# TheCacophonyProject/classifier-pipeline

Measured on AMD Instinct MI355X. Metric: CPTV frames/s end-to-end (track+classify) at 160x120, higher is better.
Workload: dtype u16/i32 track stage (f32 normalise, f64 gates); f32 crop/tile; f32 CNN (stride-1 3x3 convs of stages 2-4 (+ the stride-2 one): two fp16 planes per operand rounded to nearest (11 + 11 significand bits), power-of-two range scaling, 3 fp16 MFMAs per K step, device-side rerun in the exact split if an ac

## Files before the change

classifier-pipeline_amd/csrc/cpx_cnn_rw.hip:

```cpp
#include <hip/hip_runtime.h>

#include <algorithm>
#include <type_traits>

#include "cpx_conv_layout_core.h"
#include "cpx_kernels.h"

namespace cpx {

namespace {

typedef unsigned u32x4 __attribute__((ext_vector_type(4)));
typedef float f32x4 __attribute__((ext_vector_type(4)));
typedef _Float16 f16x2 __attribute__((ext_vector_type(2)));
typedef _Float16 f16x8 __attribute__((ext_vector_type(8)));

template <typename T>
__device__ __forceinline__ const T* at_off(const T* base, unsigned bytes) {
  return reinterpret_cast<const T*>(reinterpret_cast<const char*>(base) + bytes);
}
template <typename T>
__device__ __forceinline__ T* at_off(T* base, unsigned bytes) {
  return reinterpret_cast<T*>(reinterpret_cast<char*>(base) + bytes);
}
__device__ __forceinline__ unsigned pix_off(int y, int x, int W, int C) {
  return __umul24(__umul24((unsigned)y, (unsigned)W) + (unsigned)x, (unsigned)C);
}
__device__ __forceinline__ float relu_bits(float x) { return __int_as_float(max(__float_as_int(x), 0)); }
__device__ __forceinline__ void split_h(float a, float b, unsigned& hi, unsigned& lo) {
  f16x2 v = {(_Float16)a, (_Float16)b};
  hi = __builtin_bit_cast(unsigned, v);
  asm("v_fma_mixlo_f16 %0, %1, 1.0, -%2 op_sel:[0,0,0] op_sel_hi:[0,0,1]" : "=v"(lo) : "v"(a), "v"(hi));
  asm("v_fma_mixhi_f16 %0, %1, 1.0, -%2 op_sel:[0,0,1] op_sel_hi:[0,0,1]" : "+v"(lo) : "v"(b), "v"(hi));
}
__device__ __forceinline__ f32x4 mfma_h(u32x4 w, u32x4 x, f32x4 c) {
  return __builtin_amdgcn_mfma_f32_16x16x32_f16(__builtin_bit_cast(f16x8, w), __builtin_bit_cast(f16x8, x), c, 0, 0, 0);
}

struct RwTiles {
  unsigned long long m_tx, m_ty;
  int tiles_x, tiles_y, total;
};
template <int I, int N, typename F>
__device__ __forceinline__ void static_for(F&& f) {
  if constexpr (I < N) {
    f(std::integral_constant<int, I>{});
    static_for<I + 1, N>(f);
  }
}
__device__ __forceinline__ int div_magic(int n, unsigned long long m) { return (int)(((unsigned long long)n * m) >> 42); }

constexpr int RW_TW = 16;
constexpr int RW_CT = 256;
constexpr int RW_PPI = RW_CT / 8;
constexpr int RW_WC = 64;

template <int S, int NCH, int ROWS>
struct RwGeo {
  static constexpr int PW = 15 * S + 3, PH = (ROWS - 1) * S + 3, NPX = PH * PW;
  static constexpr int NP = (NPX * 8 + RW_CT - 1) / RW_CT;
  static constexpr int NPXP = (NP * RW_PPI + 3) / 4 * 4 + 2;
  static constexpr int BUF = 2 * 2 * NPXP * 2;
  static constexpr int STEPS = 3 * PH;
  static constexpr int CING = 32 * NCH;
  static constexpr size_t LDS = (size_t)2 * BUF * 16 + (size_t)(2 * CING + 3 * RW_WC) * sizeof(float);
};
constexpr int SC_NPXP = 258;
constexpr int SC_ITEMS = 16 * RW_TW * 8 / RW_CT;
constexpr size_t SC_LDS = (size_t)2 * 2 * SC_NPXP * 2 * 16;

template <int S, int NCH, int ROWS, bool BN, bool RES, bool SC = false>
__global__ __launch_bounds__(RW_CT) __attribute__((amdgpu_waves_per_eu(1, 1))) void conv_rw_kernel(ConvArgs a, const uint4* __restrict__ wimg, RwTiles td) {
  using G = RwGeo<S, NCH, ROWS>;
  constexpr int PW = G::PW, NPX = G::NPX, NP = G::NP, NPXP = G::NPXP, BUF = G::BUF, STEPS = G::STEPS, CING = G::CING, PH = G::PH;
  static_assert(!SC || (S == 1 && NCH == 2 && ROWS == 16 && !RES), "the fp16 shortcut is built into the stride-1 form's two-chunk stream");
  if (*a.ovf != 0) return;
  extern __shared__ __attribute__((aligned(16))) uint4 lds4[];
  uint4* s_buf = lds4;
  float* s_bn = reinterpret_cast<float*>(lds4 + 2 * BUF);
  float* s_par = s_bn + 2 * CING;
  uint4* s_sc = reinterpret_cast<uint4*>(s_par + 3 * RW_WC);
  const int tid = threadIdx.x, lane = tid & 63, wave = tid >> 6, i16 = lane & 15, q = lane >> 4;
  const int ct = wave;
  const int cout_g = a.Cout / a.groups, nhalf = cout_g / RW_WC;
  const int g = blockIdx.y / nhalf, half = blockIdx.y - g * nhalf;
  constexpr bool has_bn = BN;

  u32x4 Wr[NCH][9][2];
  {
    const u32x4* wg = reinterpret_cast<const u32x4*>(wimg) + (size_t)g * NCH * 3 * 24 * cout_g + (q * cout_g + half * RW_WC + ct * 16 + i16);
#pragma unroll
    for (int c = 0; c < NCH; ++c)
#pragma unroll
      for (int ky = 0; ky < 3; ++ky)
#pragma unroll
        for (int kx = 0; kx < 3; ++kx)
#pragma unroll
          for (int p = 0; p < 2; ++p) Wr[c][ky * 3 + kx][p] = wg[(size_t)((c * 3 + ky) * 24 + (p * 3 + kx) * 4) * cout_g];
  }
  u32x4 Wsc[2];
  if constexpr (SC) {
    const u32x4* ws = reinterpret_cast<const u32x4*>(a.sc_planes) + (size_t)g * 8 * cout_g + (q * cout_g + half * RW_WC + ct * 16 + i16);
    Wsc[0] = ws[0];
    Wsc[1] = ws[(size_t)4 * cout_g];
  }
  if (tid < CING) {
    const int ci = g * CING + tid;
    s_bn[tid] = has_bn ? a.in_scale[ci] * a.act_scale : a.act_scale;
    s_bn[CING + tid] = has_bn ? a.in_shift[ci] * a.act_scale : 0.0f;
  }
  if (tid < RW_WC) {
    const int ch = g * cout_g + half * RW_WC + tid;
    float os = a.w_unscale[ch] * a.act_unscale;
    if (a.out_scale) os *= a.out_scale[ch];
    float ob = a.out_shift ? a.out_shift[ch] : 0.0f;
    if (a.sc_in && a.sc_bias) ob += a.sc_bias[ch];
    s_par[tid] = os;
    s_par[RW_WC + tid] = ob;
    s_par[2 * RW_WC + tid] = a.w_scale[ch] * a.act_scale;
  }

  const int per_xcd = (td.total + 7) >> 3;
  auto tile_of = [&](int t) { return (t & 7) * per_xcd + (t >> 3); };
  auto decode = [&](int tile, int& n_, int& oy_, int& ox_) {
    int qd = div_magic(tile, td.m_tx);
    ox_ = (tile - qd * td.tiles_x) * RW_TW;
    tile = qd;
    qd = div_magic(tile, td.m_ty);
    oy_ = (tile - qd * td.tiles_y) * ROWS;
    n_ = qd;
  };
  int t = blockIdx.x;
  while (t < 8 * per_xcd && tile_of(t) >= td.total) t += gridDim.x;
  if (t >= 8 * per_xcd) return;
  auto advance = [&](int& n_, int& oy_, int& ox_) {
    t += gridDim.x;
    const bool more = t < 8 * per_xcd && tile_of(t) < td.total;
    if (more) decode(tile_of(t), n_, oy_, ox_);
    return more;
  };
  int n0, oy0, ox0, n1, oy1, ox1, n2, oy2, ox2;
  decode(tile_of(t), n0, oy0, ox0);

  u32x4 pre_p[NP];
  const int q8 = tid & 7;
  int ipos[NP];
#pragma unroll
  for (int i = 0; i < NP; ++i) {
    const int px = min((tid >> 3) + RW_PPI * i, NPX - 1);
    const int py = px / PW;
    ipos[i] = (py << 8) | (px - py * PW);
  }
  const unsigned st_base = (unsigned)((((q8 >> 2) * NPXP + (tid >> 3)) * 4 + (q8 & 3)) * 8);
  f32x4 psc[NCH], psh[NCH];
  const unsigned coff0 = (unsigned)(g * CING + 4 * q8);
  auto med3 = [](int x, int lo, int hi) __attribute__((always_inline)) {
    int r;
    asm("v_med3_i32 %0, %1, %2, %3" : "=v"(r) : "v"(x), "v"(lo), "s"(hi));
    return r;
  };
  const int Hm1 = a.H - 1, Wm1 = a.W - 1;
  auto issue_item = [&](const int i, const int c, const int n_, const int oy_, const int ox_) __attribute__((always_inline)) {
    const float* in_n = a.in + (size_t)n_ * a.H * a.W * a.Cin;
    const int iy = oy_ * S - a.pad_top + (ipos[i] >> 8), ix = ox_ * S - a.pad_left + (ipos[i] & 0xFF);
    const int cy = med3(iy, 0, Hm1), cx = med3(ix, 0, Wm1);
    pre_p[i] = *reinterpret_cast<const u32x4*>(at_off(in_n, (pix_off(cy, cx, a.W, a.Cin) + coff0 + (unsigned)(c * 32)) << 2));
  };
  unsigned hmax = 0u;
  auto pk_max_u16 = [](unsigned x, unsigned y) __attribute__((always_inline)) {
    unsigned r;
    asm("v_pk_max_u16 %0, %1, %2" : "=v"(r) : "v"(x), "v"(y));
    return r;
  };
  auto activate_item = [&](const int i, const int c, const int oy_, const int ox_) __attribute__((always_inline)) {
    float v[4];
#pragma unroll
    for (int j = 0; j < 4; ++j) v[j] = __fmaf_rn(__uint_as_float(pre_p[i][j]), psc[c][j], psh[c][j]);
    if (has_bn) {
#pragma unroll
      for (int j = 0; j < 4; ++j) v[j] = fmaxf(v[j], 0.0f);
    }
    const int iy = oy_ * S - a.pad_top + (ipos[i] >> 8), ix = ox_ * S - a.pad_left + (ipos[i] & 0xFF);
    const bool inside = (unsigned)iy < (unsigned)a.H && (unsigned)ix < (unsigned)a.W;
#pragma unroll
    for (int j = 0; j < 4; ++j) pre_p[i][j] = __float_as_uint(inside ? v[j] : 0.0f);
  };
  auto store_item = [&](const int i, const int bsel) __attribute__((always_inline)) {
    unsigned h0, h1, l0, l1;
    split_h(__uint_as_float(pre_p[i][0]), __uint_as_float(pre_p[i][1]), h0, l0);
    split_h(__uint_as_float(pre_p[i][2]), __uint_as_float(pre_p[i][3]), h1, l1);
    if (has_bn) hmax = pk_max_u16(pk_max_u16(hmax, h0), h1);
    else hmax = pk_max_u16(pk_max_u16(hmax, h0 & 0x7FFF7FFFu), h1 & 0x7FFF7FFFu);
    unsigned char* sp = reinterpret_cast<unsigned char*>(s_buf) + st_base;
    *reinterpret_cast<uint2*>(sp + (bsel * BUF * 16 + i * (RW_PPI * 32))) = make_uint2(h0, h1);
    *reinterpret_cast<uint2*>(sp + (bsel * BUF * 16 + 2 * NPXP * 32 + i * (RW_PPI * 32))) = make_uint2(l0, l1);
  };

  u32x4 pre_s[SC ? SC_ITEMS : 1];
  u32x4 xsh[2], xsl[2];
  const unsigned sc_st_base = (unsigned)((((q8 >> 2) * SC_NPXP + (tid >> 3)) * 4 + (q8 & 3)) * 8);
  const int sc_a_base = ((q >> 1) * SC_NPXP + i16) * 2 + (q & 1);
  auto issue_sc = [&](const int i, const int n_, const int oy_, const int ox_) __attribute__((always_inline)) {
    if constexpr (SC) {
      const float* sc_n = a.sc_in + (size_t)n_ * a.sc_H * a.sc_W * a.sc_cin;
      const int oy = min(oy_ + 2 * i + (tid >> 7), a.Ho - 1), ox = min(ox_ + ((tid >> 3) & 15), a.Wo - 1);
      pre_s[i] = *reinterpret_cast<const u32x4*>(
          at_off(sc_n, (pix_off(oy * a.sc_stride, ox * a.sc_stride, a.sc_W, a.sc_cin) + (unsigned)(g * 32 + 4 * q8)) << 2));
    }
  };
  auto store_sc = [&](const int i) __attribute__((always_inline)) {
    if constexpr (SC) {
      unsigned h0, h1, l0, l1;
      split_h(__uint_as_float(pre_s[i][0]) * a.sc_xscale, __uint_as_float(pre_s[i][1]) * a.sc_xscale, h0, l0);
      split_h(__uint_as_float(pre_s[i][2]) * a.sc_xscale, __uint_as_float(pre_s[i][3]) * a.sc_xscale, h1, l1);
      hmax = pk_max_u16(pk_max_u16(hmax, h0 & 0x7FFF7FFFu), h1 & 0x7FFF7FFFu);
      unsigned char* sp = reinterpret_cast<unsigned char*>(s_sc) + sc_st_base;
      *reinterpret_cast<uint2*>(sp + i * (RW_PPI * 32)) = make_uint2(h0, h1);
      *reinterpret_cast<uint2*>(sp + (2 * SC_NPXP * 32 + i * (RW_PPI * 32))) = make_uint2(l0, l1);
    }
  };

  f32x4 acc[ROWS];
  const int ch_l = g * cout_g + half * RW_WC + ct * 16 + 4 * q;
  auto init_acc = [&]() __attribute__((always_inline)) {
#pragma unroll
    for (int o = 0; o < ROWS; ++o) acc[o] = f32x4{0.0f, 0.0f, 0.0f, 0.0f};
  };
  f32x4 rres[RES ? ROWS : 1];
  auto issue_res = [&](const int o, const int n_, const int oy_, const int ox_) __attribute__((always_inline)) {
    if constexpr (RES) {
      const float* res_n = a.residual + (size_t)n_ * a.Ho * a.Wo * a.Cout;
      const int ox = min(ox_ + i16, a.Wo - 1), oy = min(oy_ + o, a.Ho - 1);
      rres[o] = *reinterpret_cast<const f32x4*>(at_off(res_n, (pix_off(oy, ox, a.Wo, a.Cout) + (unsigned)ch_l) << 2));
    }
  };

  const int a_base = ((q >> 1) * NPXP + S * i16) * 2 + (q & 1);
  constexpr int RW_AHEAD = 3, RW_RING = RW_AHEAD + 1;
  auto compute = [&](auto cc, auto bc, auto&& between) __attribute__((always_inline)) {
    constexpr int C = decltype(cc)::value, B = decltype(bc)::value;
    const uint4* sb = s_buf + B * BUF + a_base;
    u32x4 xh[RW_RING], xl[RW_RING];
    auto frag = [&](auto sc) __attribute__((always_inline)) {
      constexpr int s = decltype(sc)::value;
      constexpr int kx = s / PH, i = s - PH * kx, bf = s % RW_RING;
      xh[bf] = __builtin_bit_cast(u32x4, sb[(i * PW + kx) * 2]);
      xl[bf] = __builtin_bit_cast(u32x4, sb[4 * NPXP + (i * PW + kx) * 2]);
    };
    static_for<0, RW_AHEAD>(frag);
    static_for<0, STEPS>([&](auto sc) __attribute__((always_inline)) {
      constexpr int s = decltype(sc)::value;
      constexpr int kx = s / PH, i = s - PH * kx, bf = s % RW_RING;
      if constexpr (s + RW_AHEAD < STEPS) frag(std::integral_constant<int, s + RW_AHEAD>{});
      static_for<0, 3>([&](auto pc) __attribute__((always_inline)) {
        constexpr int pr = decltype(pc)::value;
        static_for<0, 3>([&](auto rc) __attribute__((always_inline)) {
          constexpr int r = decltype(rc)::value, d = i - r, o = d / S;
          if constexpr (d >= 0 && d % S == 0 && o < ROWS) {
            if constexpr (pr == 0) acc[o] = mfma_h(Wr[C][r * 3 + kx][1], xh[bf], acc[o]);
            if constexpr (pr == 1) acc[o] = mfma_h(Wr[C][r * 3 + kx][0], xl[bf], acc[o]);
            if constexpr (pr == 2) acc[o] = mfma_h(Wr[C][r * 3 + kx][0], xh[bf], acc[o]);
          }
        });
      });
      between(sc);
      __builtin_amdgcn_sched_barrier(0);
    });
  };
  auto unit = [&](auto cc, auto bc, auto ccc, auto cic, auto lastc, const int oyc, const int oxc, const int ni, const int oyi,
                  const int oxi) __attribute__((always_inline)) {
    constexpr int B = decltype(bc)::value, CC = decltype(ccc)::value, CI = decltype(cic)::value;
    constexpr bool LAST = decltype(lastc)::value;
    compute(cc, bc, [&](auto sc) __attribute__((always_inline)) {
      constexpr int s = decltype(sc)::value;
      constexpr int jlo = (s * 3 * NP + STEPS - 1) / STEPS, jhi = ((s + 1) * 3 * NP + STEPS - 1) / STEPS;
      static_for<jlo, (jhi < 3 * NP ? jhi : 3 * NP)>([&](auto jc) __attribute__((always_inline)) {
        constexpr int j = decltype(jc)::value, i = j / 3, k = j % 3;
        if constexpr (k == 0) activate_item(i, CC, oyc, oxc);
        if constexpr (k == 1) store_item(i, B ^ 1);
        if constexpr (k == 2) issue_item(i, CI, ni, oyi, oxi);
      });
      if constexpr (SC && !LAST) {
        constexpr int klo = (s * SC_ITEMS + STEPS - 1) / STEPS, khi = ((s + 1) * SC_ITEMS + STEPS - 1) / STEPS;
        static_for<klo, (khi < SC_ITEMS ? khi : SC_ITEMS)>([&](auto kc) __attribute__((always_inline)) { store_sc(decltype(kc)::value); });
      }
      if constexpr (SC && LAST) {
        if constexpr (s % 3 == 0 && s >= 3 && s / 3 - 1 < ROWS) {
          constexpr int o = s / 3 - 1;
          acc[o] = mfma_h(Wsc[1], xsh[o & 1], acc[o]);
          acc[o] = mfma_h(Wsc[0], xsl[o & 1], acc[o]);
          acc[o] = mfma_h(Wsc[0], xsh[o & 1], acc[o]);
        }
        if constexpr (s % 3 == 0 && s / 3 < ROWS) {
          constexpr int o = s / 3;
          xsh[o & 1] = __builtin_bit_cast(u32x4, s_sc[sc_a_base + o * 2 * RW_TW]);
          xsl[o & 1] = __builtin_bit_cast(u32x4, s_sc[sc_a_base + 4 * SC_NPXP + o * 2 * RW_TW]);
        }
        constexpr int klo = (s * SC_ITEMS + STEPS - 1) / STEPS, khi = ((s + 1) * SC_ITEMS + STEPS - 1) / STEPS;
        static_for<klo, (khi < SC_ITEMS ? khi : SC_ITEMS)>([&](auto kc) __attribute__((always_inline)) { issue_sc(decltype(kc)::value, ni, oyi, oxi); });
      }
      if constexpr (LAST && RES) {
        constexpr int olo = (s * ROWS + STEPS - 1) / STEPS, ohi = ((s + 1) * ROWS + STEPS - 1) / STEPS;
        static_for<olo, (ohi < ROWS ? ohi : ROWS)>([&](auto oc) __attribute__((always_inline)) { issue_res(decltype(oc)::value, n0, oy0, ox0); });
      }
    });
  };

  auto finish = [&](const int n_, const int oy_, const int ox_) __attribute__((always_inline)) {
    const int ox = min(ox_ + i16, a.Wo - 1);
    if (!SC && a.sc_in) {
      const int sc_cg = a.sc_cin / a.groups;
      const float* wsc = a.sc_w + ((size_t)g * sc_cg + q) * cout_g + half * RW_WC + ct * 16 + i16;
      const float ss = s_par[2 * RW_WC + ct * 16 + i16];
      const float* sc_n = a.sc_in + (size_t)n_ * a.sc_H * a.sc_W * a.sc_cin + g * sc_cg + q;
      for (int k4 = 0; k4 < sc_cg; k4 += 4) {
        const float ws = wsc[(size_t)k4 * cout_g] * ss;
#pragma unroll
        for (int o = 0; o < ROWS; ++o) {
          const int oy = min(oy_ + o, a.Ho - 1);
          const float xs = sc_n[((size_t)(oy * a.sc_stride) * a.sc_W + ox * a.sc_stride) * a.sc_cin + k4];
          acc[o] = __builtin_amdgcn_mfma_f32_16x16x4f32(ws, xs, acc[o], 0, 0, 0);
        }
      }
    }
    float* out_n = a.out + (size_t)n_ * a.Ho * a.Wo * a.Cout;
    const f32x4 os = *reinterpret_cast<const f32x4*>(s_par + ct * 16 + 4 * q);
    const f32x4 ob = *reinterpret_cast<const f32x4*>(s_par + RW_WC + ct * 16 + 4 * q);
    const bool xok = ox_ + i16 < a.Wo;
    const unsigned off0 = (pix_off(min(oy_, a.Ho - 1), ox, a.Wo, a.Cout) + (unsigned)ch_l) << 2;
    const unsigned row_bytes = (unsigned)(a.Wo * a.Cout) << 2;
    const bool whole = oy_ + ROWS <= a.Ho;
    auto row = [&](const int o, const bool ok, const unsigned off) __attribute__((always_inline)) {
      f32x4 v;
#pragma unroll
      for (int j = 0; j < 4; ++j) v[j] = __fmaf_rn(acc[o][j], os[j], ob[j]);
      if constexpr (RES) v += rres[o];
      if (a.relu) {
        asm volatile("");
        v.x = relu_bits(v.x); v.y = relu_bits(v.y); v.z = relu_bits(v.z); v.w = relu_bits(v.w);
      }
      if (ok) *reinterpret_cast<f32x4*>(at_off(out_n, off)) = v;
    };
    if (whole) {
#pragma unroll
      for (int o = 0; o < ROWS; ++o) row(o, xok, off0 + (unsigned)o * row_bytes);
    } else {
#pragma unroll
      for (int o = 0; o < ROWS; ++o) row(o, xok && oy_ + o < a.Ho, off0 + (unsigned)min(o, a.Ho - 1 - oy_) * row_bytes);
    }
  };

#pragma unroll
  for (int i = 0; i < NP; ++i) issue_item(i, 0, n0, oy0, ox0);
  __syncthreads();
#pragma unroll
  for (int c = 0; c < NCH; ++c) {
    psc[c] = *reinterpret_cast<const f32x4*>(s_bn + c * 32 + 4 * q8);
    psh[c] = *reinterpret_cast<const f32x4*>(s_bn + CING + c * 32 + 4 * q8);
  }
#pragma unroll
  for (int i = 0; i < NP; ++i) {
    activate_item(i, 0, oy0, ox0);
    store_item(i, 0);
  }
  using I0 = std::integral_constant<int, 0>;
  using I1 = std::integral_constant<int, 1>;
  using Yes = std::integral_constant<bool, true>;
  using No = std::integral_constant<bool, false>;
  if constexpr (NCH == 2) {
#pragma unroll
    for (int i = 0; i < NP; ++i) issue_item(i, 1, n0, oy0, ox0);
    if constexpr (SC) {
#pragma unroll
      for (int i = 0; i < SC_ITEMS; ++i) issue_sc(i, n0, oy0, ox0);
    }
    init_acc();
    for (;;) {
      n1 = n0; oy1 = oy0; ox1 = ox0;
      const bool more = advance(n1, oy1, ox1);
      __syncthreads();
      unit(I0{}, I0{}, I1{}, I0{}, No{}, oy0, ox0, n1, oy1, ox1);
      __syncthreads();
      unit(I1{}, I1{}, I0{}, I1{}, Yes{}, oy1, ox1, n1, oy1, ox1);
      finish(n0, oy0, ox0);
      if (!more) break;
      n0 = n1; oy0 = oy1; ox0 = ox1;
      init_acc();
    }
  } else {
    n1 = n0; oy1 = oy0; ox1 = ox0;
    bool more1 = advance(n1, oy1, ox1);
#pragma unroll
    for (int i = 0; i < NP; ++i) issue_item(i, 0, n1, oy1, ox1);
    init_acc();
    for (;;) {
      n2 = n1; oy2 = oy1; ox2 = ox1;
      bool more2 = more1 && advance(n2, oy2, ox2);
      __syncthreads();
      unit(I0{}, I0{}, I0{}, I0{}, Yes{}, oy1, ox1, n2, oy2, ox2);
      finish(n0, oy0, ox0);
      if (!more1) break;
      n0 = n1; oy0 = oy1; ox0 = ox1; n1 = n2; oy1 = oy2; ox1 = ox2; more1 = more2;
      init_acc();
      n2 = n1; oy2 = oy1; ox2 = ox1;
      more2 = more1 && advance(n2, oy2, ox2);
      __syncthreads();
      unit(I0{}, I1{}, I0{}, I0{}, Yes{}, oy1, ox1, n2, oy2, ox2);
      finish(n0, oy0, ox0);
      if (!more1) break;
      n0 = n1; oy0 = oy1; ox0 = ox1; n1 = n2; oy1 = oy2; ox1 = ox2; more1 = more2;
      init_acc();
    }
  }
  if ((hmax & 0x7FFFu) >= 0x7C00u || ((hmax >> 16) & 0x7FFFu) >= 0x7C00u) atomicOr(a.ovf, 1);
}

__global__ __launch_bounds__(256) void split_shortcut_kernel(const float* __restrict__ w, uint4* __restrict__ out, int groups, int cin_g,
                                                             int cout_g, const float* __restrict__ wscale, float factor) {
  const int nch = cin_g / 32;
  const int total = groups * nch * 4 * cout_g;
  const int idx = blockIdx.x * blockDim.x + threadIdx.x;
  if (idx >= total) return;
  const int col = idx % cout_g;
  int r = idx / cout_g;
  const int qq = r & 3;
  r >>= 2;
  const int chunk = r % nch, g = r / nch;
  const float f = wscale[g * cout_g + col] * factor;
  float v[8];
#pragma unroll
  for (int j = 0; j < 8; ++j) v[j] = w[((size_t)g * cin_g + chunk * 32 + 8 * qq + j) * cout_g + col] * f;
  uint4 hi, lo;
  split_h(v[0], v[1], hi.x, lo.x);
  split_h(v[2], v[3], hi.y, lo.y);
  split_h(v[4], v[5], hi.z, lo.z);
  split_h(v[6], v[7], hi.w, lo.w);
  const size_t base = (size_t)(g * nch + chunk) * 8 * cout_g + (size_t)qq * cout_g + col;
  out[base] = hi;
  out[base + (size_t)4 * cout_g] = lo;
}

}

bool conv_shortcut_planes_layer(const ConvArgs& second, int sc_cin_g) {
  if (conv_rw_kind(second) == 1) return sc_cin_g == 32;
  return second.ksize == 3 && second.stride == 1 && second.groups >= 1 && second.Cin == second.Cout &&
         second.Cout == 128 * second.groups && sc_cin_g == 64;
}
size_t conv_shortcut_image_bytes(int groups, int cin_g, int cout_g) { return (size_t)groups * (cin_g / 32) * 8 * cout_g * 16; }
void launch_split_shortcut(const float* sc_w, void* img, int groups, int cin_g, int cout_g, const float* w_scale, float factor,
                           hipStream_t s) {
  const int total = groups * (cin_g / 32) * 4 * cout_g;
  hipLaunchKernelGGL(split_shortcut_kernel, dim3((unsigned)((total + 255) / 256)), dim3(256), 0, s, sc_w, reinterpret_cast<uint4*>(img),
                     groups, cin_g, cout_g, w_scale, factor);
}

int conv_rw_kind(const ConvArgs& a) { return conv_rw_kind_of(conv_shape_of(a)); }
bool conv_rw_layer(const ConvArgs& a) { return conv_rw_kind(a) == 1; }

namespace {
template <int S, int NCH, int ROWS, bool BN, bool RES, bool SC = false>
int launch_rw_t(const ConvArgs& a, const uint4* wimg, hipStream_t s) {
  using G = RwGeo<S, NCH, ROWS>;
  constexpr size_t LDS = G::LDS + (SC ? SC_LDS : 0);
  static_assert(LDS <= 160 * 1024 - 1024, "two chunk buffers (and the shortcut's operand) must fit the CU's LDS");
  RwTiles td{};
  if (const int rc = fill_tiles(td, (a.Wo + RW_TW - 1) / RW_TW, (a.Ho + ROWS - 1) / ROWS, a.N, TILES_PERSISTENT)) return rc;
  static bool lds_ready[64];
  if (!cpx_dyn_lds_ready(reinterpret_cast<const void*>(conv_rw_kernel<S, NCH, ROWS, BN, RES, SC>), lds_ready, 160 * 1024 - 1024)) return -1;
  const int cus = cpx_device_cus();
  if (cus == 0) return -1;
  const int ny = a.groups * ((a.Cout / a.groups) / RW_WC);
  const int gx = persistent_grid_x(cus, ny, td.total);
  hipLaunchKernelGGL((conv_rw_kernel<S, NCH, ROWS, BN, RES, SC>), dim3((unsigned)gx, (unsigned)ny), dim3(RW_CT), LDS, s, a, wimg, td);
  return 0;
}
}

int launch_conv_rw(const ConvArgs& a, const void* wimg, hipStream_t s) {
  const int kind = conv_rw_kind(a);
  if (!kind || !a.half || a.planes != 2 || a.ovf == nullptr || a.in_planes || a.out_planes) return -2;
  if ((long long)a.H * a.W >= (1 << 24) || (long long)a.Ho * a.Wo >= (1 << 24)) return -3;
  if (a.sc_in && ((a.sc_cin / a.groups) & 3)) return -2;
  const uint4* wi = reinterpret_cast<const uint4*>(wimg);
  const bool bn = a.in_scale != nullptr, res = a.residual != nullptr;
  if (kind == 1) {
    if (a.pad_top != 1 || a.pad_left != 1 || a.H != a.Ho || a.W != a.Wo) return -2;
    if (a.sc_in && a.sc_planes) {
      if (bn || res || !conv_shortcut_planes_layer(a, a.sc_cin / a.groups) || a.sc_stride < 1 || !(a.sc_xscale > 0.0f) ||
          (a.sc_H - 1) / a.sc_stride + 1 != a.Ho || (a.sc_W - 1) / a.sc_stride + 1 != a.Wo)
        return -2;
      if ((long long)a.sc_H * a.sc_W >= (1 << 24) || (long long)a.sc_H * a.sc_W * a.sc_cin >= (1ll << 30)) return -3;
      return launch_rw_t<1, 2, 16, false, false, true>(a, wi, s);
    }
    if (bn && res) return launch_rw_t<1, 2, 16, true, true>(a, wi, s);
    if (bn) return launch_rw_t<1, 2, 16, true, false>(a, wi, s);
    if (res) return launch_rw_t<1, 2, 16, false, true>(a, wi, s);
    return launch_rw_t<1, 2, 16, false, false>(a, wi, s);
  }
  if (res || a.sc_in || a.pad_top < 0 || a.pad_top > 1 || a.pad_left < 0 || a.pad_left > 1) return -2;
  if (kind == 2) return bn ? launch_rw_t<2, 1, 8, true, false>(a, wi, s) : launch_rw_t<2, 1, 8, false, false>(a, wi, s);
  return bn ? launch_rw_t<3, 2, 4, true, false>(a, wi, s) : launch_rw_t<3, 2, 4, false, false>(a, wi, s);
}

}
```

classifier-pipeline_amd/csrc/cpx_conv_layout_core.h:

```cpp
#pragma once
#include <stddef.h>

#include <algorithm>

namespace cpx {

struct ConvShape { int groups, cin_g, cout_g, ksize, stride; };
template <class Args>
ConvShape conv_shape_of(const Args& a) {
  if (a.groups < 1 || a.Cin % a.groups || a.Cout % a.groups) return ConvShape{};
  return ConvShape{a.groups, a.Cin / a.groups, a.Cout / a.groups, a.ksize, a.stride};
}

enum class ConvClass { Unsupported, Plain, Flat, Wide, C8, Stride2Rw, Rw3 };

inline ConvClass conv_class(const ConvShape& s) {
  if (s.ksize != 3) return ConvClass::Unsupported;
  if (s.stride == 3 && s.cin_g == 64 && s.cout_g == 128) return ConvClass::Rw3;
  if (s.stride == 2 && s.cin_g == 32 && s.cout_g == 64) return ConvClass::Stride2Rw;
  if (s.stride == 1 && s.cin_g == 8 && s.cout_g == 32) return ConvClass::C8;
  const bool c32_64 = s.cout_g == 32 || s.cout_g == 64;
  if (s.stride == 1 && (s.cin_g == 32 || s.cin_g == 64) && c32_64) return ConvClass::Wide;
  if (s.cin_g < 16 || s.cin_g % 16) return ConvClass::Unsupported;
  if ((s.stride == 1 && s.cout_g == 128) || (s.stride == 2 && s.cout_g == 64)) return ConvClass::Flat;
  return s.stride == 1 && c32_64 ? ConvClass::Plain : ConvClass::Unsupported;
}
inline int conv_rw_kind_of(const ConvShape& s) {
  switch (conv_class(s)) {
    case ConvClass::Wide: return s.cin_g == 64 && s.cout_g == 64 ? 1 : 0;
    case ConvClass::Stride2Rw: return 2;
    case ConvClass::Rw3: return 3;
    default: return 0;
  }
}

struct WeightImages {
  static constexpr size_t absent = ~(size_t)0;
  static constexpr size_t C8_HALF_ENTRIES = 3 * 2 * 4 * 32;
  ConvClass cls = ConvClass::Unsupported;
  int chunk = 0;
  size_t planes3 = absent, planes2 = absent, half = absent, scales = absent, rw_half = absent, bytes = 0;

  static WeightImages of(const ConvShape& s) {
    WeightImages l;
    l.cls = conv_class(s);
    if (l.cls == ConvClass::Unsupported) return l;
    const auto put = [&l](size_t& image, size_t size) { image = l.bytes; l.bytes += size; };
    const size_t row = (size_t)s.cout_g * 16;
    const size_t scales = ((size_t)2 * s.groups * s.cout_g * sizeof(float) + 15) / 16 * 16;
    if (l.cls == ConvClass::C8) {
      put(l.planes3, (size_t)s.groups * 30 * row);
      put(l.half, (size_t)s.groups * C8_HALF_ENTRIES * 16);
      put(l.scales, scales);
      return l;
    }
    l.chunk = l.cls == ConvClass::Wide || l.cls == ConvClass::Rw3 ? 32 : 16;
    const auto image = [&](int planes) { return (size_t)s.groups * (s.cin_g / l.chunk) * (9 * l.chunk / 8 * planes) * row; };
    if (l.cls != ConvClass::Rw3) put(l.planes3, image(3));
    if (l.cls == ConvClass::Plain) return l;
    if (l.cls != ConvClass::Rw3) put(l.planes2, image(2));
    put(l.half, image(2));
    put(l.scales, scales);
    if (l.cls == ConvClass::Stride2Rw) put(l.rw_half, image(2));
    return l;
  }
};

constexpr int TILE_AXIS_LIMIT = 4096;
constexpr long long TILES_PER_LAUNCH = 1ll << 22;
constexpr long long TILES_PERSISTENT = (1ll << 22) - 8;
inline unsigned long long tile_magic(int d) { return (1ull << 42) / (unsigned long long)d + 1; }

template <class Tiles>
int fill_tiles(Tiles& td, int tiles_x, int tiles_y, long long n, long long limit) {
  if (tiles_x < 1 || tiles_y < 1 || tiles_x >= TILE_AXIS_LIMIT || tiles_y >= TILE_AXIS_LIMIT) return -3;
  const long long total = (long long)tiles_x * tiles_y * n;
  if (total >= limit) return -3;
  td.tiles_x = tiles_x, td.m_tx = tile_magic(tiles_x);
  td.tiles_y = tiles_y, td.m_ty = tile_magic(tiles_y);
  td.total = (int)total;
  return 0;
}
template <class Tiles>
int fill_tiles(Tiles& td, int tiles_x, int tiles_y, long long n, int nsplit, long long limit) {
  if (nsplit < 1 || nsplit >= TILE_AXIS_LIMIT) return -3;
  td.nsplit = nsplit, td.m_nsplit = tile_magic(nsplit);
  return fill_tiles(td, tiles_x, tiles_y, n * nsplit, limit);
}

inline int persistent_grid_x(int cus, int ny, long long tiles) {
  const int gx = std::max(8, cus / std::max(ny, 1) / 8 * 8);
  return (int)std::min<long long>(gx, (tiles + 7) / 8 * 8);
}

}
```

Before: 3.106 million.

## Give each wave two output-channel tiles in the stride-3 row-window conv

For the stride-3 layer (64->128 channels), each wave now computes two 16-channel output tiles, so one block covers all 128 channels and each staged input fragment feeds twice as many MFMAs. This halves the grid in y and removes the duplicate input staging and fp16 splitting across blocks. To keep register pressure manageable it shortens the fragment prefetch ring, issues fragment loads after the products, and computes item positions arithmetically. It also adds a CPX_RW_GRID environment override for the persistent grid size. The risk is higher VGPR use (doubled weight and accumulator registers) and fewer blocks in flight.

```diff
diff --git a/classifier-pipeline_amd/csrc/cpx_cnn_rw.hip b/classifier-pipeline_amd/csrc/cpx_cnn_rw.hip
--- a/classifier-pipeline_amd/csrc/cpx_cnn_rw.hip
+++ b/classifier-pipeline_amd/csrc/cpx_cnn_rw.hip
@@ -1,6 +1,7 @@
 #include <hip/hip_runtime.h>
 
 #include <algorithm>
+#include <cstdlib>
 #include <type_traits>
 
 #include "cpx_conv_layout_core.h"
@@ -63,7 +64,8 @@
   static constexpr int BUF = 2 * 2 * NPXP * 2;
   static constexpr int STEPS = 3 * PH;
   static constexpr int CING = 32 * NCH;
-  static constexpr size_t LDS = (size_t)2 * BUF * 16 + (size_t)(2 * CING + 3 * RW_WC) * sizeof(float);
+  static constexpr int CTW = S == 3 ? 2 : 1, WC = RW_WC * CTW;
+  static constexpr size_t LDS = (size_t)2 * BUF * 16 + (size_t)(2 * CING + 3 * WC) * sizeof(float);
 };
 constexpr int SC_NPXP = 258;
 constexpr int SC_ITEMS = 16 * RW_TW * 8 / RW_CT;
@@ -73,34 +75,38 @@
 __global__ __launch_bounds__(RW_CT) __attribute__((amdgpu_waves_per_eu(1, 1))) void conv_rw_kernel(ConvArgs a, const uint4* __restrict__ wimg, RwTiles td) {
   using G = RwGeo<S, NCH, ROWS>;
   constexpr int PW = G::PW, NPX = G::NPX, NP = G::NP, NPXP = G::NPXP, BUF = G::BUF, STEPS = G::STEPS, CING = G::CING, PH = G::PH;
+  constexpr int CTW = G::CTW, WC = G::WC;
+  static_assert(CTW == 1 || (!RES && !SC), "two channel tiles per wave: the stride-3 layer has neither residual nor shortcut");
   static_assert(!SC || (S == 1 && NCH == 2 && ROWS == 16 && !RES), "the fp16 shortcut is built into the stride-1 form's two-chunk stream");
   if (*a.ovf != 0) return;
   extern __shared__ __attribute__((aligned(16))) uint4 lds4[];
   uint4* s_buf = lds4;
   float* s_bn = reinterpret_cast<float*>(lds4 + 2 * BUF);
   float* s_par = s_bn + 2 * CING;
-  uint4* s_sc = reinterpret_cast<uint4*>(s_par + 3 * RW_WC);
+  uint4* s_sc = reinterpret_cast<uint4*>(s_par + 3 * WC);
   const int tid = threadIdx.x, lane = tid & 63, wave = tid >> 6, i16 = lane & 15, q = lane >> 4;
-  const int ct = wave;
-  const int cout_g = a.Cout / a.groups, nhalf = cout_g / RW_WC;
+  const int ct = wave * CTW;
+  const int cout_g = a.Cout / a.groups, nhalf = cout_g / WC;
   const int g = blockIdx.y / nhalf, half = blockIdx.y - g * nhalf;
   constexpr bool has_bn = BN;
 
-  u32x4 Wr[NCH][9][2];
+  u32x4 Wr[CTW][NCH][9][2];
   {
-    const u32x4* wg = reinterpret_cast<const u32x4*>(wimg) + (size_t)g * NCH * 3 * 24 * cout_g + (q * cout_g + half * RW_WC + ct * 16 + i16);
-#pragma unroll
-    for (int c = 0; c < NCH; ++c)
-#pragma unroll
-      for (int ky = 0; ky < 3; ++ky)
-#pragma unroll
-        for (int kx = 0; kx < 3; ++kx)
-#pragma unroll
-          for (int p = 0; p < 2; ++p) Wr[c][ky * 3 + kx][p] = wg[(size_t)((c * 3 + ky) * 24 + (p * 3 + kx) * 4) * cout_g];
+    const u32x4* wg = reinterpret_cast<const u32x4*>(wimg) + (size_t)g * NCH * 3 * 24 * cout_g + (q * cout_g + half * WC + ct * 16 + i16);
+#pragma unroll
+    for (int w = 0; w < CTW; ++w)
+#pragma unroll
+      for (int c = 0; c < NCH; ++c)
+#pragma unroll
+        for (int ky = 0; ky < 3; ++ky)
+#pragma unroll
+          for (int kx = 0; kx < 3; ++kx)
+#pragma unroll
+            for (int p = 0; p < 2; ++p) Wr[w][c][ky * 3 + kx][p] = wg[(size_t)((c * 3 + ky) * 24 + (p * 3 + kx) * 4) * cout_g + w * 16];
   }
   u32x4 Wsc[2];
   if constexpr (SC) {
-    const u32x4* ws = reinterpret_cast<const u32x4*>(a.sc_planes) + (size_t)g * 8 * cout_g + (q * cout_g + half * RW_WC + ct * 16 + i16);
+    const u32x4* ws = reinterpret_cast<const u32x4*>(a.sc_planes) + (size_t)g * 8 * cout_g + (q * cout_g + half * WC + ct * 16 + i16);
     Wsc[0] = ws[0];
     Wsc[1] = ws[(size_t)4 * cout_g];
   }
@@ -109,15 +115,15 @@
     s_bn[tid] = has_bn ? a.in_scale[ci] * a.act_scale : a.act_scale;
     s_bn[CING + tid] = has_bn ? a.in_shift[ci] * a.act_scale : 0.0f;
   }
-  if (tid < RW_WC) {
-    const int ch = g * cout_g + half * RW_WC + tid;
+  if (tid < WC) {
+    const int ch = g * cout_g + half * WC + tid;
     float os = a.w_unscale[ch] * a.act_unscale;
     if (a.out_scale) os *= a.out_scale[ch];
     float ob = a.out_shift ? a.out_shift[ch] : 0.0f;
     if (a.sc_in && a.sc_bias) ob += a.sc_bias[ch];
     s_par[tid] = os;
-    s_par[RW_WC + tid] = ob;
-    s_par[2 * RW_WC + tid] = a.w_scale[ch] * a.act_scale;
+    s_par[WC + tid] = ob;
+    s_par[2 * WC + tid] = a.w_scale[ch] * a.act_scale;
   }
 
   const int per_xcd = (td.total + 7) >> 3;
@@ -144,26 +150,36 @@
 
   u32x4 pre_p[NP];
   const int q8 = tid & 7;
-  int ipos[NP];
-#pragma unroll
-  for (int i = 0; i < NP; ++i) {
-    const int px = min((tid >> 3) + RW_PPI * i, NPX - 1);
-    const int py = px / PW;
-    ipos[i] = (py << 8) | (px - py * PW);
-  }
+  constexpr bool IPOS3 = S == 3;
+  static_assert(!IPOS3 || (PW == 48 && RW_PPI == 32 && NP * RW_PPI == NPX), "item i = pixel (tid >> 3) + 32 i of a 48-pixel row, none past the patch");
+  int ipos[IPOS3 ? 2 : NP];
+  if constexpr (IPOS3) {
+    const int px0 = tid >> 3;
+    ipos[0] = px0;
+    ipos[1] = px0 < 16 ? px0 + 32 : (1 << 8) | (px0 - 16);
+  } else {
+#pragma unroll
+    for (int i = 0; i < NP; ++i) {
+      const int px = min((tid >> 3) + RW_PPI * i, NPX - 1);
+      const int py = px / PW;
+      ipos[i] = (py << 8) | (px - py * PW);
+    }
+  }
+  auto item_pos = [&](const int i) __attribute__((always_inline)) { return IPOS3 ? ipos[i % 3 == 1] + ((2 * i / 3) << 8) + (i % 3 == 2 ? 16 : 0) : ipos[i]; };
   const unsigned st_base = (unsigned)((((q8 >> 2) * NPXP + (tid >> 3)) * 4 + (q8 & 3)) * 8);
   f32x4 psc[NCH], psh[NCH];
   const unsigned coff0 = (unsigned)(g * CING + 4 * q8);
-  auto med3 = [](int x, int lo, int hi) __attribute__((always_inline)) {
+  auto clamp0 = [](int x, int hi) __attribute__((always_inline)) {
     int r;
-    asm("v_med3_i32 %0, %1, %2, %3" : "=v"(r) : "v"(x), "v"(lo), "s"(hi));
+    asm("v_med3_i32 %0, %1, 0, %2" : "=v"(r) : "v"(x), "s"(hi));
     return r;
   };
   const int Hm1 = a.H - 1, Wm1 = a.W - 1;
   auto issue_item = [&](const int i, const int c, const int n_, const int oy_, const int ox_) __attribute__((always_inline)) {
     const float* in_n = a.in + (size_t)n_ * a.H * a.W * a.Cin;
-    const int iy = oy_ * S - a.pad_top + (ipos[i] >> 8), ix = ox_ * S - a.pad_left + (ipos[i] & 0xFF);
-    const int cy = med3(iy, 0, Hm1), cx = med3(ix, 0, Wm1);
+    const int ip = item_pos(i);
+    const int iy = oy_ * S - a.pad_top + (ip >> 8), ix = ox_ * S - a.pad_left + (ip & 0xFF);
+    const int cy = clamp0(iy, Hm1), cx = clamp0(ix, Wm1);
     pre_p[i] = *reinterpret_cast<const u32x4*>(at_off(in_n, (pix_off(cy, cx, a.W, a.Cin) + coff0 + (unsigned)(c * 32)) << 2));
   };
   unsigned hmax = 0u;
@@ -180,20 +196,21 @@
 #pragma unroll
       for (int j = 0; j < 4; ++j) v[j] = fmaxf(v[j], 0.0f);
     }
-    const int iy = oy_ * S - a.pad_top + (ipos[i] >> 8), ix = ox_ * S - a.pad_left + (ipos[i] & 0xFF);
+    const int ip = item_pos(i);
+    const int iy = oy_ * S - a.pad_top + (ip >> 8), ix = ox_ * S - a.pad_left + (ip & 0xFF);
     const bool inside = (unsigned)iy < (unsigned)a.H && (unsigned)ix < (unsigned)a.W;
 #pragma unroll
     for (int j = 0; j < 4; ++j) pre_p[i][j] = __float_as_uint(inside ? v[j] : 0.0f);
   };
-  auto store_item = [&](const int i, const int bsel) __attribute__((always_inline)) {
+  auto store_item = [&](const int i, const unsigned boff) __attribute__((always_inline)) {
     unsigned h0, h1, l0, l1;
     split_h(__uint_as_float(pre_p[i][0]), __uint_as_float(pre_p[i][1]), h0, l0);
     split_h(__uint_as_float(pre_p[i][2]), __uint_as_float(pre_p[i][3]), h1, l1);
     if (has_bn) hmax = pk_max_u16(pk_max_u16(hmax, h0), h1);
     else hmax = pk_max_u16(pk_max_u16(hmax, h0 & 0x7FFF7FFFu), h1 & 0x7FFF7FFFu);
     unsigned char* sp = reinterpret_cast<unsigned char*>(s_buf) + st_base;
-    *reinterpret_cast<uint2*>(sp + (bsel * BUF * 16 + i * (RW_PPI * 32))) = make_uint2(h0, h1);
-    *reinterpret_cast<uint2*>(sp + (bsel * BUF * 16 + 2 * NPXP * 32 + i * (RW_PPI * 32))) = make_uint2(l0, l1);
+    *reinterpret_cast<uint2*>(sp + (boff + i * (RW_PPI * 32))) = make_uint2(h0, h1);
+    *reinterpret_cast<uint2*>(sp + (boff + 2 * NPXP * 32 + i * (RW_PPI * 32))) = make_uint2(l0, l1);
   };
 
   u32x4 pre_s[SC ? SC_ITEMS : 1];
@@ -220,11 +237,13 @@
     }
   };
 
-  f32x4 acc[ROWS];
-  const int ch_l = g * cout_g + half * RW_WC + ct * 16 + 4 * q;
+  f32x4 acc[CTW][ROWS];
+  const int ch_l = g * cout_g + half * WC + ct * 16 + 4 * q;
   auto init_acc = [&]() __attribute__((always_inline)) {
 #pragma unroll
-    for (int o = 0; o < ROWS; ++o) acc[o] = f32x4{0.0f, 0.0f, 0.0f, 0.0f};
+    for (int w = 0; w < CTW; ++w)
+#pragma unroll
+      for (int o = 0; o < ROWS; ++o) acc[w][o] = f32x4{0.0f, 0.0f, 0.0f, 0.0f};
   };
   f32x4 rres[RES ? ROWS : 1];
   auto issue_res = [&](const int o, const int n_, const int oy_, const int ox_) __attribute__((always_inline)) {
@@ -236,9 +255,28 @@
   };
 
   const int a_base = ((q >> 1) * NPXP + S * i16) * 2 + (q & 1);
-  constexpr int RW_AHEAD = 3, RW_RING = RW_AHEAD + 1;
+  constexpr bool FRAG_AFTER = CTW == 2;
+  constexpr int RW_AHEAD = S == 3 ? 2 : 3, RW_RING = FRAG_AFTER ? RW_AHEAD : RW_AHEAD + 1;
+  auto products = [&](auto cc, auto sc, const u32x4& h, const u32x4& l) __attribute__((always_inline)) {
+    constexpr int C = decltype(cc)::value, s = decltype(sc)::value;
+    constexpr int kx = s / PH, i = s - PH * kx;
+    static_for<0, 3>([&](auto pc) __attribute__((always_inline)) {
+      constexpr int pr = decltype(pc)::value;
+      static_for<0, 3>([&](auto rc) __attribute__((always_inline)) {
+        constexpr int r = decltype(rc)::value, d = i - r, o = d / S;
+        if constexpr (d >= 0 && d % S == 0 && o < ROWS) {
+          static_for<0, CTW>([&](auto wc) __attribute__((always_inline)) {
+            constexpr int w = decltype(wc)::value;
+            if constexpr (pr == 0) acc[w][o] = mfma_h(Wr[w][C][r * 3 + kx][1], h, acc[w][o]);
+            if constexpr (pr == 1) acc[w][o] = mfma_h(Wr[w][C][r * 3 + kx][0], l, acc[w][o]);
+            if constexpr (pr == 2) acc[w][o] = mfma_h(Wr[w][C][r * 3 + kx][0], h, acc[w][o]);
+          });
+        }
+      });
+    });
+  };
   auto compute = [&](auto cc, auto bc, auto&& between) __attribute__((always_inline)) {
-    constexpr int C = decltype(cc)::value, B = decltype(bc)::value;
+    constexpr int B = decltype(bc)::value;
     const uint4* sb = s_buf + B * BUF + a_base;
     u32x4 xh[RW_RING], xl[RW_RING];
     auto frag = [&](auto sc) __attribute__((always_inline)) {
@@ -250,19 +288,10 @@
     static_for<0, RW_AHEAD>(frag);
     static_for<0, STEPS>([&](auto sc) __attribute__((always_inline)) {
       constexpr int s = decltype(sc)::value;
-      constexpr int kx = s / PH, i = s - PH * kx, bf = s % RW_RING;
-      if constexpr (s + RW_AHEAD < STEPS) frag(std::integral_constant<int, s + RW_AHEAD>{});
-      static_for<0, 3>([&](auto pc) __attribute__((always_inline)) {
-        constexpr int pr = decltype(pc)::value;
-        static_for<0, 3>([&](auto rc) __attribute__((always_inline)) {
-          constexpr int r = decltype(rc)::value, d = i - r, o = d / S;
-          if constexpr (d >= 0 && d % S == 0 && o < ROWS) {
-            if constexpr (pr == 0) acc[o] = mfma_h(Wr[C][r * 3 + kx][1], xh[bf], acc[o]);
-            if constexpr (pr == 1) acc[o] = mfma_h(Wr[C][r * 3 + kx][0], xl[bf], acc[o]);
-            if constexpr (pr == 2) acc[o] = mfma_h(Wr[C][r * 3 + kx][0], xh[bf], acc[o]);
-          }
-        });
-      });
+      constexpr int bf = s % RW_RING;
+      if constexpr (!FRAG_AFTER && s + RW_AHEAD < STEPS) frag(std::integral_constant<int, s + RW_AHEAD>{});
+      products(cc, sc, xh[bf], xl[bf]);
+      if constexpr (FRAG_AFTER && s + RW_AHEAD < STEPS) frag(std::integral_constant<int, s + RW_AHEAD>{});
       between(sc);
       __builtin_amdgcn_sched_barrier(0);
     });
@@ -271,13 +300,17 @@
                   const int oxi) __attribute__((always_inline)) {
     constexpr int B = decltype(bc)::value, CC = decltype(ccc)::value, CI = decltype(cic)::value;
     constexpr bool LAST = decltype(lastc)::value;
+    if constexpr (CTW == 2) {
+      psc[CC] = *reinterpret_cast<const f32x4*>(s_bn + CC * 32 + 4 * q8);
+      psh[CC] = *reinterpret_cast<const f32x4*>(s_bn + CING + CC * 32 + 4 * q8);
+    }
     compute(cc, bc, [&](auto sc) __attribute__((always_inline)) {
       constexpr int s = decltype(sc)::value;
       constexpr int jlo = (s * 3 * NP + STEPS - 1) / STEPS, jhi = ((s + 1) * 3 * NP + STEPS - 1) / STEPS;
       static_for<jlo, (jhi < 3 * NP ? jhi : 3 * NP)>([&](auto jc) __attribute__((always_inline)) {
         constexpr int j = decltype(jc)::value, i = j / 3, k = j % 3;
         if constexpr (k == 0) activate_item(i, CC, oyc, oxc);
-        if constexpr (k == 1) store_item(i, B ^ 1);
+        if constexpr (k == 1) store_item(i, (unsigned)((B ^ 1) * BUF * 16));
         if constexpr (k == 2) issue_item(i, CI, ni, oyi, oxi);
       });
       if constexpr (SC && !LAST) {
@@ -287,9 +320,9 @@
       if constexpr (SC && LAST) {
         if constexpr (s % 3 == 0 && s >= 3 && s / 3 - 1 < ROWS) {
           constexpr int o = s / 3 - 1;
-          acc[o] = mfma_h(Wsc[1], xsh[o & 1], acc[o]);
-          acc[o] = mfma_h(Wsc[0], xsl[o & 1], acc[o]);
-          acc[o] = mfma_h(Wsc[0], xsh[o & 1], acc[o]);
+          acc[0][o] = mfma_h(Wsc[1], xsh[o & 1], acc[0][o]);
+          acc[0][o] = mfma_h(Wsc[0], xsl[o & 1], acc[0][o]);
+          acc[0][o] = mfma_h(Wsc[0], xsh[o & 1], acc[0][o]);
         }
         if constexpr (s % 3 == 0 && s / 3 < ROWS) {
           constexpr int o = s / 3;
@@ -307,11 +340,15 @@
   };
 
   auto finish = [&](const int n_, const int oy_, const int ox_) __attribute__((always_inline)) {
+    int ft = tid;
+    if constexpr (CTW == 2) asm volatile("" : "+v"(ft));
+    const int i16 = ft & 15, q = (ft >> 4) & 3, ct = (ft >> 6) * CTW;
+    const int ch_l = g * cout_g + half * WC + ct * 16 + 4 * q;
     const int ox = min(ox_ + i16, a.Wo - 1);
-    if (!SC && a.sc_in) {
+    if (!SC && CTW == 1 && a.sc_in) {
       const int sc_cg = a.sc_cin / a.groups;
-      const float* wsc = a.sc_w + ((size_t)g * sc_cg + q) * cout_g + half * RW_WC + ct * 16 + i16;
-      const float ss = s_par[2 * RW_WC + ct * 16 + i16];
+      const float* wsc = a.sc_w + ((size_t)g * sc_cg + q) * cout_g + half * WC + ct * 16 + i16;
+      const float ss = s_par[2 * WC + ct * 16 + i16];
       const float* sc_n = a.sc_in + (size_t)n_ * a.sc_H * a.sc_W * a.sc_cin + g * sc_cg + q;
       for (int k4 = 0; k4 < sc_cg; k4 += 4) {
         const float ws = wsc[(size_t)k4 * cout_g] * ss;
@@ -319,35 +356,38 @@
         for (int o = 0; o < ROWS; ++o) {
           const int oy = min(oy_ + o, a.Ho - 1);
           const float xs = sc_n[((size_t)(oy * a.sc_stride) * a.sc_W + ox * a.sc_stride) * a.sc_cin + k4];
-          acc[o] = __builtin_amdgcn_mfma_f32_16x16x4f32(ws, xs, acc[o], 0, 0, 0);
+          acc[0][o] = __builtin_amdgcn_mfma_f32_16x16x4f32(ws, xs, acc[0][o], 0, 0, 0);
         }
       }
     }
     float* out_n = a.out + (size_t)n_ * a.Ho * a.Wo * a.Cout;
-    const f32x4 os = *reinterpret_cast<const f32x4*>(s_par + ct * 16 + 4 * q);
-    const f32x4 ob = *reinterpret_cast<const f32x4*>(s_par + RW_WC + ct * 16 + 4 * q);
     const bool xok = ox_ + i16 < a.Wo;
     const unsigned off0 = (pix_off(min(oy_, a.Ho - 1), ox, a.Wo, a.Cout) + (unsigned)ch_l) << 2;
     const unsigned row_bytes = (unsigned)(a.Wo * a.Cout) << 2;
     const bool whole = oy_ + ROWS <= a.Ho;
-    auto row = [&](const int o, const bool ok, const unsigned off) __attribute__((always_inline)) {
-      f32x4 v;
-#pragma unroll
-      for (int j = 0; j < 4; ++j) v[j] = __fmaf_rn(acc[o][j], os[j], ob[j]);
-      if constexpr (RES) v += rres[o];
-      if (a.relu) {
-        asm volatile("");
-        v.x = relu_bits(v.x); v.y = relu_bits(v.y); v.z = relu_bits(v.z); v.w = relu_bits(v.w);
+    static_for<0, CTW>([&](auto wc) __attribute__((always_inline)) {
+      constexpr int w = decltype(wc)::value;
+      const f32x4 os = *reinterpret_cast<const f32x4*>(s_par + (ct + w) * 16 + 4 * q);
+      const f32x4 ob = *reinterpret_cast<const f32x4*>(s_par + WC + (ct + w) * 16 + 4 * q);
+      auto row = [&](const int o, const bool ok, const unsigned off) __attribute__((always_inline)) {
+        f32x4 v;
+#pragma unroll
+        for (int j = 0; j < 4; ++j) v[j] = __fmaf_rn(acc[w][o][j], os[j], ob[j]);
+        if constexpr (RES) v += rres[o];
+        if (a.relu) {
+          asm volatile("");
+          v.x = relu_bits(v.x); v.y = relu_bits(v.y); v.z = relu_bits(v.z); v.w = relu_bits(v.w);
+        }
+        if (ok) *reinterpret_cast<f32x4*>(at_off(out_n, off + (unsigned)(w * 64))) = v;
+      };
+      if (whole) {
+#pragma unroll
+        for (int o = 0; o < ROWS; ++o) row(o, xok, off0 + (unsigned)o * row_bytes);
+      } else {
+#pragma unroll
+        for (int o = 0; o < ROWS; ++o) row(o, xok && oy_ + o < a.Ho, off0 + (unsigned)min(o, a.Ho - 1 - oy_) * row_bytes);
       }
-      if (ok) *reinterpret_cast<f32x4*>(at_off(out_n, off)) = v;
-    };
-    if (whole) {
-#pragma unroll
-      for (int o = 0; o < ROWS; ++o) row(o, xok, off0 + (unsigned)o * row_bytes);
-    } else {
-#pragma unroll
-      for (int o = 0; o < ROWS; ++o) row(o, xok && oy_ + o < a.Ho, off0 + (unsigned)min(o, a.Ho - 1 - oy_) * row_bytes);
-    }
+    });
   };
 
 #pragma unroll
@@ -361,7 +401,7 @@
 #pragma unroll
   for (int i = 0; i < NP; ++i) {
     activate_item(i, 0, oy0, ox0);
-    store_item(i, 0);
+    store_item(i, 0u);
   }
   using I0 = std::integral_constant<int, 0>;
   using I1 = std::integral_constant<int, 1>;
@@ -470,8 +510,10 @@
   if (!cpx_dyn_lds_ready(reinterpret_cast<const void*>(conv_rw_kernel<S, NCH, ROWS, BN, RES, SC>), lds_ready, 160 * 1024 - 1024)) return -1;
   const int cus = cpx_device_cus();
   if (cus == 0) return -1;
-  const int ny = a.groups * ((a.Cout / a.groups) / RW_WC);
-  const int gx = persistent_grid_x(cus, ny, td.total);
+  const int ny = conv_rw_grid_y(conv_shape_of(a));
+  if (ny < 1 || ny * G::WC != a.Cout) return -2;
+  const char* e = std::getenv("CPX_RW_GRID");
+  const int gx = e ? persistent_grid_x(std::atoi(e), 1, td.total) : persistent_grid_x(cus, ny, td.total);
   hipLaunchKernelGGL((conv_rw_kernel<S, NCH, ROWS, BN, RES, SC>), dim3((unsigned)gx, (unsigned)ny), dim3(RW_CT), LDS, s, a, wimg, td);
   return 0;
 }
diff --git a/classifier-pipeline_amd/csrc/cpx_conv_layout_core.h b/classifier-pipeline_amd/csrc/cpx_conv_layout_core.h
--- a/classifier-pipeline_amd/csrc/cpx_conv_layout_core.h
+++ b/classifier-pipeline_amd/csrc/cpx_conv_layout_core.h
@@ -32,6 +32,12 @@
     case ConvClass::Rw3: return 3;
     default: return 0;
   }
+}
+
+inline int conv_rw_channels_of(int kind) { return kind == 3 ? 128 : kind ? 64 : 0; }
+inline int conv_rw_grid_y(const ConvShape& s) {
+  const int wc = conv_rw_channels_of(conv_rw_kind_of(s));
+  return wc && s.cout_g % wc == 0 ? s.groups * (s.cout_g / wc) : 0;
 }
 
 struct WeightImages {
```

Result: no change. 3.133 million, median of 6 (+0.9%).
